# openxrlab/xrslam

Hardware: AMD Instinct MI355X
Metric: frames/sec, full per-frame hot path (KLT tracker + sliding-window VI-BA), one sequence per GPU (higher is better)
Workload: dtype u8/i16 images, f32 LK with exact i64 reductions, f64 BA

## Files before the change

xrslam_amd/csrc/ba_api.hip:

```cpp
#include "../../include/xrslam_hip.h"
#include "ba_kernels.hip.h"
#include "ba_chain.hip.h"
#include "ba_plan.hpp"
#include "ba_stage.hpp"
#include "marg_kernels.hip.h"
#include "cov_kernels.hip.h"
#include "host/covariance.hpp"
#include "common.hip.h"
#include "group.hip.h"

#include <cstdlib>
#include <chrono>
#include <algorithm>
#include <cmath>
#include <cstring>
#include <limits>
#include <vector>

using namespace xrhip;

namespace {

struct Grow {
    size_t headroom, floor;
// ... 81 lines not shown
        bool pending = false;
        int K = 0, victim = 0, R = 0;
        std::vector<double> lin;
        int *dst = nullptr;
        double *lam = nullptr;
    } marg;
    int preint_pending = 0;
    PreintScratch preint_o{};
    int preint_deferred = 0, preint_def_jac = 0, preint_def_cov = 0;
    bool profiling = false;
    struct Timed {
        hipEvent_t e0, e1;
        double flops_fixed, flops_per_trial;
        int iter_before;
    };
    std::vector<Timed> pending;
    struct TimedChain {
        hipEvent_t e0, e1;
        double bytes;
    };
    std::vector<TimedChain> pending_chain;
    std::vector<std::pair<hipEvent_t, hipEvent_t>> free_events;
    xrhip_ba_stats stats = {0, 0, 0.0, 0, 0.0, 0, 0, 0.0, 0.0, 0};
    DevBuf<> cov_dev;
    hipEvent_t cov_ev[5] = {nullptr, nullptr, nullptr, nullptr, nullptr};
    double cov_ms[4] = {0.0, 0.0, 0.0, 0.0};
    const TinyArgs *tiny_args = nullptr;
    hipStream_t stream2 = nullptr;
    hipEvent_t ev_mid = nullptr, ev_spec = nullptr;
    hipEvent_t ev_marg = nullptr;
    DevBuf<> work_spec;
    bool spec_outstanding = false;
    long spec_launched = 0, spec_taken = 0;
    const uint4 *stage_src = nullptr;
    uint4 *stage_dst = nullptr;
    size_t stage_n16 = 0;
    void (*overlap_fn)(void *) = nullptr;
    void *overlap_arg = nullptr;
    PinnedBuf<double> h_out;
    int lds_limit = 150 * 1024;
    int schur_mode = 0;
    SolvePlan plan;
};

static int ensure_arena(xrhip_ba *c, size_t in_bytes, size_t work_bytes, size_t out_doubles) {
    int rc = c->in.dev.reserve(in_bytes, GROW_DOUBLE_1M);
    if (!rc) rc = c->in.host.reserve(in_bytes, GROW_DOUBLE_1M);
    if (!rc) rc = c->work.reserve(work_bytes, GROW_DOUBLE_1M);
    if (!rc) rc = c->h_out.reserve(sizeof(double) * out_doubles, GROW_DOUBLE);
    return rc;
}

static int validate(const xrhip_ba_problem *P) {
    if (!P || P->n_frames <= 0 || !P->frame_state || !P->frame_fix) return xr_fail(XRHIP_EINVAL, "xrhip_ba_solve: frames missing");
    if (P->n_landmarks < 0 || P->n_obs < 0 || P->n_rot < 0 || P->n_imu < 0 || P->prior_n < 0)
        return xr_fail(XRHIP_EINVAL, "xrhip_ba_solve: negative count");
    for (int o = 0; o < P->n_obs; ++o)
        if (P->obs_tgt[o] < 0 || P->obs_tgt[o] >= P->n_frames || P->obs_ref[o] < 0 || P->obs_ref[o] >= P->n_frames ||
            P->obs_lm[o] < 0 || P->obs_lm[o] >= P->n_landmarks || P->obs_tgt[o] == P->obs_ref[o])
            return xr_fail(XRHIP_EINVAL, "xrhip_ba_solve: observation index out of range");
    for (int o = 0; o < P->n_rot; ++o)
        if (P->rot_tgt[o] < 0 || P->rot_tgt[o] >= P->n_frames || P->rot_ref[o] < 0 || P->rot_ref[o] >= P->n_frames)
            return xr_fail(XRHIP_EINVAL, "xrhip_ba_solve: rotation factor index out of range");
    for (int k = 0; k < P->n_imu; ++k)
        if (P->imu_i[k] < 0 || P->imu_i[k] >= P->n_frames || P->imu_j[k] < 0 || P->imu_j[k] >= P->n_frames ||
            P->imu_i[k] == P->imu_j[k])
// ... 195 lines not shown
    c->stage_n16 = (lay.in_bytes + 15) / 16;
    return defer_copy ? XRHIP_OK : launch_stage_copy(c, c->stream);
}

static int landmark_vision_blocks(const BaDims &d) { return d.lm_rows + d.F * d.F * VIS_CH; }
static int assemble_blocks(const BaDims &d) { return (d.n * d.n + 255) / 256; }
static size_t lin_all_lds(const BaDims &d) { return sizeof(double) * (size_t)std::max(d.np, 1); }
static int schur_aux_blocks(const BaDims &d) {
    const int tiles = d.PF / 16;
    const int nrest = sred_rest_blocks(d);
    return nrest + (d.nla ? tiles * tiles + aux_quad_blocks_n(d.n, d.L) + aux_wog_blocks(d.F) : aux_quad_blocks_n(d.n, d.L)) + 1;
}

static void launch_linearize(xrhip_ba *c, const Staged &st, bool for_solver) {
    hipStream_t s = c->stream;
    const BaDims &d = st.d;
    const BaPtrs &p = st.p;
    hipLaunchKernelGGL(kb_lin_all, dim3(lin_all_blocks(d.M, d.MR, d.NI, d.np)), dim3(256), lin_all_lds(d), s, d, p, st.cam, st.imu, st.sx, st.sy);
    hipLaunchKernelGGL(kb_landmark_vision, dim3(landmark_vision_blocks(d)), dim3(64), 0, s, d, p);
    if (for_solver && st.pl.route == ROUTE_SMALL_MID) return;
    hipLaunchKernelGGL(kb_assemble, dim3(assemble_blocks(d)), dim3(256), 0, s, d, p);
    if (for_solver) hipLaunchKernelGGL(kb_prepare, dim3(1), dim3(256), 0, s, d, p);
    else hipLaunchKernelGGL(kb_sum_cost, dim3(1), dim3(256), 0, s, d, p);
}

constexpr int LINEARIZE_LAUNCHES = 4;

static void launch_schur_aux(const Staged &st, hipStream_t s) {
    hipLaunchKernelGGL(kb_schur_aux, dim3(schur_aux_blocks(st.d)), dim3(256), 0, s, st.d, st.p);
}
static void launch_prior_lambda(const Staged &st, hipStream_t s) {
    hipLaunchKernelGGL(kb_prior_lambda, dim3(prior_lambda_blocks(st.d.np)), dim3(256), 0, s, st.d.np, st.p.pS, st.p.pLam, st.p.pinfo, st.p.pc0);
}
static void launch_trials_wide(const Staged &st, hipStream_t s, int seq, int first, int mode) {
    hipLaunchKernelGGL(kb_trials_wide, dim3(WIDE_G), dim3(256), st.pl.wide_lds, s, st.d, st.p, st.cam, st.imu, st.sx, st.sy, seq, first, mode);
}

static int take_event_pair(xrhip_ba *c, hipEvent_t *e0, hipEvent_t *e1) {
    if (!c->free_events.empty()) {
        *e0 = c->free_events.back().first;
        *e1 = c->free_events.back().second;
        c->free_events.pop_back();
    } else {
        XR_HIP(hipEventCreate(e0));
        XR_HIP(hipEventCreate(e1));
    }
    return XRHIP_OK;
}

static int launch_solve_try(xrhip_ba *c, const Staged &st, bool prepare, int mode, int seq, bool skip_front = false,
                            const BaPtrs *spec_set = nullptr) {
    const BaDims &d = st.d;
    const BaPtrs &p = st.p;
    const SolvePlan &pl = st.pl;
    const bool mark_mid = spec_set != nullptr;
    const int commit = (spec_set && skip_front) ? 1 : 0;
    double *state2 = spec_set ? static_cast<double *>(spec_set->state) : nullptr;
    double *depth2 = spec_set ? static_cast<double *>(spec_set->depth) : nullptr;
    BaCtl *ctl2 = spec_set ? static_cast<BaCtl *>(spec_set->ctl) : nullptr;
    hipStream_t s = c->stream;
    const bool mid = pl.route == ROUTE_SMALL_MID;
    if (!skip_front) {
        if (mid) hipLaunchKernelGGL(kb_small_mid, dim3(1), dim3(256), 0, s, d, p, prepare ? 0 : 1);
        if (!mid && prepare) hipLaunchKernelGGL(kb_prepare, dim3(1), dim3(256), 0, s, d, p);
        if (!mid) launch_schur_aux(st, s);
    }
    const size_t lds = pl.try_lds;
    const int use_lds = pl.use_lds, wide = pl.wide_trials ? 1 : 0;
// ... 8 lines not shown
    else if (pl.block == 256)
        hipLaunchKernelGGL((kb_solve_try<256, false>), dim3(1), dim3(256), lds, s, d, p, st.cam, st.imu, st.sx, st.sy, use_lds, mode, seq, wide,
                           (double *)nullptr, (double *)nullptr, (BaCtl *)nullptr, 0);
    else
        hipLaunchKernelGGL((kb_solve_try<512, false>), dim3(1), dim3(512), lds, s, d, p, st.cam, st.imu, st.sx, st.sy, use_lds, mode, seq, wide,
                           (double *)nullptr, (double *)nullptr, (BaCtl *)nullptr, 0);
    XR_HIP(hipGetLastError());
    if (c->profiling) XR_HIP(hipEventRecord(e1, s));
    if (pl.wide_first) {
        hipStream_t ts = s;
        if (mark_mid) {
            XR_HIP(hipEventRecord(c->ev_mid, s));
            XR_HIP(hipStreamWaitEvent(c->stream2, c->ev_mid, 0));
            ts = c->stream2;
        }
        launch_trials_wide(st, ts, seq, 1, mode);
        XR_HIP(hipGetLastError());
    }
    if (c->profiling) {
        const double na = d.na;
        c->pending.push_back({e0, e1, na * na * na / 3.0 + 2.0 * na * na,
                              pl.wide_first ? 0.0 : 450.0 * d.M + 3000.0 * d.NI + 2.0 * (double)d.np * d.np, -1});
    }
    c->stats.n_solve_try++;
    return XRHIP_OK;
}

static void run_overlap(xrhip_ba *c) {
    if (!c->overlap_fn) return;
    void (*fn)(void *) = c->overlap_fn;
    c->overlap_fn = nullptr;
    fn(c->overlap_arg);
}
static int wait_mailbox(xrhip_ba *c, int seq, hipStream_t publisher = nullptr, GroupRequest *rq = nullptr) {
    run_overlap(c);
    return wait_flag(c->h_seq, seq, publisher ? publisher : c->stream, rq, "xrhip_ba_solve");
}

static long long g_kprof[32];
static void kprof_accumulate(const BaCtl &ctl, int na) {
    static const int min_na = std::getenv("XRHIP_KPROF_MIN_NA") ? std::atoi(std::getenv("XRHIP_KPROF_MIN_NA")) : 0;
    static const int max_na = std::getenv("XRHIP_KPROF_MAX_NA") ? std::atoi(std::getenv("XRHIP_KPROF_MAX_NA")) : 1 << 30;
    if (na < min_na || na > max_na) return;
    for (int i = 0; i < 31; ++i) g_kprof[i] += ctl.prof[i];
    g_kprof[31] += 1;
}

extern "C" {

static void ba_resolve_pending(xrhip_ba *c) {
    for (auto &t : c->pending) {
        float ms = 0.f;
        if (hipEventSynchronize(t.e1) == hipSuccess && hipEventElapsedTime(&ms, t.e0, t.e1) == hipSuccess) {
            c->stats.ms_solve_try += ms;
            c->stats.n_timed += 1;
            c->stats.flops_solve_try += t.flops_fixed + t.flops_per_trial * std::max(t.iter_before, 0);
        }
        c->free_events.push_back({t.e0, t.e1});
    }
    c->pending.clear();
    for (auto &t : c->pending_chain) {
        float ms = 0.f;
        if (hipEventSynchronize(t.e1) == hipSuccess && hipEventElapsedTime(&ms, t.e0, t.e1) == hipSuccess) {
            c->stats.ms_chain += ms;
            c->stats.n_chain_timed += 1;
            c->stats.bytes_chain += t.bytes;
        }
        c->free_events.push_back({t.e0, t.e1});
    }
// ... 3 lines not shown
int xrhip_ba_set_profiling(xrhip_ba *c, int enable) {
    if (!c) return xr_fail(XRHIP_EINVAL, "xrhip_ba_set_profiling: null context");
    if (!enable) ba_resolve_pending(c);
    c->profiling = enable != 0;
    return XRHIP_OK;
}

int xrhip_ba_get_stats(xrhip_ba *c, xrhip_ba_stats *out, int reset) {
    if (!c || !out) return xr_fail(XRHIP_EINVAL, "xrhip_ba_get_stats: null argument");
    ba_resolve_pending(c);
    *out = c->stats;
    if (reset) c->stats = {0, 0, 0.0, 0, 0.0, 0, 0, 0.0, 0.0, 0};
    return XRHIP_OK;
}

void xrhip_debug_kprof(long long *out32, int reset) {
    for (int i = 0; i < 32; ++i) {
        if (out32) out32[i] = g_kprof[i];
        if (reset) g_kprof[i] = 0;
    }
}

int xrhip_ba_create(int max_frames, int max_landmarks, int max_obs, xrhip_ba **out) {
    if (!out || max_frames <= 0 || max_landmarks < 0 || max_obs < 0) return xr_fail(XRHIP_EINVAL, "xrhip_ba_create: bad arguments");
    int rc = xr_require_device();
    if (rc) return rc;
    xrhip_ba *c = new xrhip_ba();
    XR_HIP(hipGetDevice(&c->device));
    XR_HIP(hipStreamCreateWithFlags(&c->stream, hipStreamNonBlocking));
    XR_HIP(hipStreamCreateWithFlags(&c->stream2, hipStreamNonBlocking));
    XR_HIP(hipEventCreateWithFlags(&c->ev_mid, hipEventDisableTiming));
    XR_HIP(hipEventCreateWithFlags(&c->ev_spec, hipEventDisableTiming));
    XR_HIP(hipHostMalloc(&c->h_ctl, sizeof(BaCtl), hipHostMallocDefault));
    XR_HIP(hipHostMalloc(&c->h_seq, 64, hipHostMallocDefault));
    *c->h_seq = 0;
    XR_HIP(hipFuncSetAttribute((const void *)kb_solve_try<512, true>, hipFuncAttributeMaxDynamicSharedMemorySize, c->lds_limit));
    XR_HIP(hipFuncSetAttribute((const void *)kb_solve_try<512, false>, hipFuncAttributeMaxDynamicSharedMemorySize, c->lds_limit));
    XR_HIP(hipFuncSetAttribute((const void *)kb_solve_try<256, false>, hipFuncAttributeMaxDynamicSharedMemorySize, c->lds_limit));
    XR_HIP(hipFuncSetAttribute((const void *)kb_chain, hipFuncAttributeMaxDynamicSharedMemorySize, c->lds_limit));
    XR_HIP(hipFuncSetAttribute((const void *)kb_trials_wide, hipFuncAttributeMaxDynamicSharedMemorySize, c->lds_limit));
    XR_HIP(hipFuncSetAttribute((const void *)kw_solve_try, hipFuncAttributeMaxDynamicSharedMemorySize, c->lds_limit));
    XR_HIP(hipFuncSetAttribute((const void *)kw_trials_wide, hipFuncAttributeMaxDynamicSharedMemorySize, c->lds_limit));
    XR_HIP(hipFuncSetAttribute((const void *)km_chol, hipFuncAttributeMaxDynamicSharedMemorySize, c->lds_limit));
    XR_HIP(hipFuncSetAttribute((const void *)km_jacobi, hipFuncAttributeMaxDynamicSharedMemorySize, c->lds_limit));
    size_t in_guess = (size_t)max_obs * 96 + (size_t)max_frames * max_frames * 15 * 15 * 8 + (size_t)max_frames * 3000 + 65536;
    rc = ensure_arena(c, in_guess, in_guess * 4, (size_t)16 * max_frames + max_landmarks + 8);
    if (rc) return rc;
    *out = c;
    return XRHIP_OK;
}

int xrhip_ba_join_group(xrhip_ba *c, xrhip_group *g) {
    if (!c) return xr_fail(XRHIP_EINVAL, "xrhip_ba_join_group: null context");
    if (c->group == g) return XRHIP_OK;
    if (g && group_device(g) != c->device)
        return xr_fail(XRHIP_EINVAL, "xrhip_ba_join_group: the context and the group live on different devices");
    if (c->preint_pending) {
        if (c->preint_rq) {
            int rc = group_wait_launched(c->preint_rq);
            if (rc) return rc;
        }
        XR_HIP(hipStreamSynchronize(c->preint_stream ? c->preint_stream : c->stream));
        c->preint_rq = nullptr;
        c->preint_stream = c->stream;
    }
    XR_HIP(hipStreamSynchronize(c->stream));
    if (c->group) {
        int rc = group_drain(c->group, GQ_CHAIN, c);
        if (!rc) rc = group_drain(c->group, GQ_PREINT, c);
        if (!rc) rc = group_drain(c->group, GQ_WINDOW, c);
        if (rc) return rc;
        group_member_remove(c->group, false);
    }
    c->group = g;
    if (g) group_member_add(g, false);
    return XRHIP_OK;
}

void xrhip_ba_destroy(xrhip_ba *c) {
    if (!c) return;
    if (c->begun.active) xrhip_ba_solve_abort(c);
    if (c->group) {
        xrhip_ba_preintegrate_cancel(c);
        xrhip_ba_join_group(c, nullptr);
    }
    hipStreamSynchronize(c->stream);
    if (c->stream2) hipStreamSynchronize(c->stream2);
    if (std::getenv("XRHIP_HOSTPROF") && c->spec_launched)
        std::fprintf(stderr, "[hostprof] speculative linearisations: %ld launched, %ld taken\n", c->spec_launched, c->spec_taken);
    c->work_spec.release();
    c->cov_dev.release();
    for (hipEvent_t e : c->cov_ev)
        if (e) hipEventDestroy(e);
    if (c->ev_mid) hipEventDestroy(c->ev_mid);
    if (c->ev_marg) hipEventDestroy(c->ev_marg);
    if (c->ev_spec) hipEventDestroy(c->ev_spec);
    if (c->stream2) hipStreamDestroy(c->stream2);
    c->in.dev.release();
    c->in.host.release();
    c->work.release();
    c->work2.release();
    c->h_stage.release();
    hipHostFree(c->h_ctl);
    hipHostFree(c->h_seq);
    ba_resolve_pending(c);
    for (auto &e : c->free_events) {
        hipEventDestroy(e.first);
        hipEventDestroy(e.second);
    }
    c->h_out.release();
    hipStreamDestroy(c->stream);
    delete c;
}

static int preint_launch_deferred(xrhip_ba *c, const xrhip_ba_problem *P, const double *state_dev);
static int preint_fill_deferred(xrhip_ba *c, const xrhip_ba_problem *P, const double *state_dev, PreintArgs *out, bool *have);

static int ba_solve_impl(xrhip_ba *c, const xrhip_ba_problem *P, xrhip_ba_summary *summary);
int xrhip_ba_solve(xrhip_ba *c, const xrhip_ba_problem *P, xrhip_ba_summary *summary) {
    if (!c) return xr_fail(XRHIP_EINVAL, "xrhip_ba_solve: null context");
    if (c->begun.active) return xr_fail(XRHIP_ESTATE, "xrhip_ba_solve: a solve begun on this context has not been collected (xrhip_ba_solve_end)");
    const int rc = ba_solve_impl(c, P, summary);
// ... 211 lines not shown
    return XRHIP_OK;
}

int xrhip_ba_solve_chained(xrhip_ba *c1, const xrhip_ba_problem *P1, xrhip_ba_summary *s1, int link_first, xrhip_ba *c2,
                           const xrhip_ba_problem *P2, xrhip_ba_summary *s2, int link_second, void (*host_work)(void *), void *arg) {
    if (!c1 || !c2 || c1 == c2 || !P1 || !P2) return xr_fail(XRHIP_EINVAL, "xrhip_ba_solve_chained: two distinct contexts and two problems are needed");
    int rc = validate(P1);
    if (!rc) rc = validate(P2);
    if (rc) return rc;
    if (link_first < 0 || link_first >= P1->n_frames || link_second < 0 || link_second >= P2->n_frames)
        return xr_fail(XRHIP_EINVAL, "xrhip_ba_solve_chained: linked frame is not a frame of its problem");
    const int begun = xrhip_ba_solve_begin(c1, P1);
    if (begun < 0) return begun;
    if (begun == 0) {
        rc = xrhip_ba_solve_overlapped(c1, P1, s1, host_work, arg);
        if (rc) return rc;
        std::memcpy(P2->frame_state + 16 * (size_t)link_second, P1->frame_state + 16 * (size_t)link_first, sizeof(double) * 16);
        return xrhip_ba_solve(c2, P2, s2);
    }
    rc = xrhip_ba_solve_linked(c2, P2, s2, link_second, c1, link_first, host_work, arg);
    const int rc1 = xrhip_ba_solve_end(c1, s1);
    return rc ? rc : rc1;
}

struct RoundIssuer {
    enum Form { OWN, SPEC, GROUP };
    xrhip_ba *c;
    Staged &st;
    Form form;
    hipStream_t wstream;
    Staged st2{};
    bool spec_ready = false;
    bool first = true, relin = true;

    int begin_spec() {
        const int rc = c->work_spec.reserve(c->work.cap + spec_extra_bytes(st.d), GROW_EXACT);
        if (rc) return rc;
        st2 = st;
        st2.p = spec_set(st.p, st.d, c->work.p, c->work_spec.p, c->work.cap);
        return XRHIP_OK;
    }
    int request(int kind, int seq, int mode) {
        int r = group_wait_launched(&c->rq_window);
        if (r) return r;
        const BaDims &d = st.d;
        WindowPayload &wp = c->a_window;
        wp.e = WinEntry{c->tiny_args, lin_all_blocks(d.M, d.MR, d.NI, d.np), landmark_vision_blocks(d), assemble_blocks(d), schur_aux_blocks(d),
                        st.pl.use_lds, mode, seq, 1};
        wp.relin = relin;
        wp.with_stage = first;
        wp.stage = StageArgs{c->stage_src, c->stage_dst, c->stage_n16};
        wp.np = d.np;
        wp.pS = st.p.pS;
        wp.pLam = st.p.pLam;
        wp.pinfo = st.p.pinfo;
        wp.pc0 = st.p.pc0;
        wp.lds_lin = lin_all_lds(d);
        wp.lds_solve = st.pl.try_lds;
        wp.lds_wide = st.pl.wide_lds;
        c->rq_window.kind = kind;
        c->rq_window.owner = c;
        c->rq_window.payload = &wp;
        first = false;
        return group_submit(c->group, GQ_WINDOW, &c->rq_window);
    }
    int round(bool relinearise, int mode, int seq) {
        relin = relinearise;
        if (form == GROUP) return request(GK_WROUND, seq, mode);
        int rc;
        if (spec_ready) {
            rc = launch_solve_try(c, st, false, mode, seq, true, &st2.p);
        } else {
            if (relinearise) launch_linearize(c, st, true);
            rc = launch_solve_try(c, st, !relinearise, mode, seq, false, form == SPEC ? &st2.p : nullptr);
        }
        if (rc) return rc;
        spec_ready = false;
        if (form == SPEC) {
            launch_linearize(c, st2, true);
            launch_schur_aux(st2, c->stream);
            XR_HIP(hipGetLastError());
            c->spec_launched++;
        }
        return XRHIP_OK;
    }
    int trials(int seq) {
        if (form == GROUP) return request(GK_WTRIALS, seq, 0);
        launch_trials_wide(st, form == SPEC ? c->stream2 : c->stream, seq, 0, 0);
        XR_HIP(hipGetLastError());
        return XRHIP_OK;
    }
    int wait(int seq) {
        if (form == GROUP) return wait_mailbox(c, seq, wstream, &c->rq_window);
        return wait_mailbox(c, seq, form == SPEC ? c->stream2 : nullptr);
    }
    void costed(int n_trials) {
        if (c->profiling && form != GROUP && !c->pending.empty()) c->pending.back().iter_before = n_trials;
    }
    void take_speculation() {
        if (form != SPEC) return;
        swap_lin_sets(st.p, st2.p);
        spec_ready = true;
        c->spec_taken++;
    }
};

static int ba_solve_impl(xrhip_ba *c, const xrhip_ba_problem *P, xrhip_ba_summary *summary) {
    int rc = validate(P);
    if (rc) return rc;
    rc = preint_deferred_check(c, P);
    if (rc) return rc;
    c->plan = SolvePlan{};
    c->plan.F = P->n_frames;
    bool any_free = any_free_block(P);
    if (!any_free) {
        std::vector<char> used(std::max(P->n_landmarks, 1), 0);
        for (int o = 0; o < P->n_obs; ++o) used[P->obs_lm[o]] = 1;
        for (int l = 0; l < P->n_landmarks; ++l)
            if (used[l] && !(P->landmark_fix && P->landmark_fix[l])) any_free = true;
    }
    if (!any_free) {
        if (summary) {
            std::memset(summary, 0, sizeof(*summary));
            summary->termination = XRHIP_BA_CONVERGENCE;
            summary->usable = 1;
        }
        return preint_launch_deferred(c, P, nullptr);
// ... 27 lines not shown
    const BaSwitches &sw = ba_switches();
    const bool wbatch = c->group && !sw.group_no_window_batch && pl.wide_first && d.nla > 0 && !sw.group_spec;
    const bool spec = !sw.no_spec && pl.wide_first && !(c->group && !sw.group_spec);
    if (!wbatch) {
        rc = launch_stage_copy(c, c->stream);
        if (rc) return rc;
    }
    if (!d.nla) st.d.lm_rows = 0;
    if (d.np && !wbatch) launch_prior_lambda(st, c->stream);
    RoundIssuer rounds{c, st, wbatch ? RoundIssuer::GROUP : spec ? RoundIssuer::SPEC : RoundIssuer::OWN,
                       wbatch ? group_stream(c->group, GQ_WINDOW) : nullptr};
    bool done = false;
    struct BusyElsewhere {
        xrhip_group *g;
        explicit BusyElsewhere(xrhip_group *gg) : g(gg) { group_busy_elsewhere(g, 1); }
        ~BusyElsewhere() { group_busy_elsewhere(g, -1); }
    } busy_elsewhere(c->group);
    if (pl.route == ROUTE_TINY) {
        const int seq = ++c->seq;
        hipLaunchKernelGGL(kb_tiny, dim3(1), dim3(256), pl.try_lds, c->stream, c->tiny_args, pl.use_lds, seq, 4 * (P->max_iterations + 8));
        XR_HIP(hipGetLastError());
        rc = wait_mailbox(c, seq);
        if (rc) return rc;
        if (c->h_ctl->status != ST_DONE) return xr_fail(XRHIP_ESTATE, "xrhip_ba_solve: trust-region loop did not terminate");
        c->stats.n_tiny++;
        done = true;
    }
    if (rounds.form == RoundIssuer::SPEC) {
        rc = rounds.begin_spec();
        if (rc) return rc;
    }
    bool relinearise = true;
    int mode = 1, iter_seen = 0;
    auto trials_since = [&]() {
        const int it_now = c->h_ctl->iteration, trials = std::max(0, it_now - iter_seen);
        iter_seen = it_now;
        c->stats.n_trials += trials;
        return trials;
    };
    for (int guard = 0; guard < 4 * (P->max_iterations + 8) && !done; ++guard) {
        const int seq = ++c->seq;
        rc = rounds.round(relinearise, mode, seq);
        if (!rc) rc = rounds.wait(seq);
        if (rc) return rc;
        const bool first_batch_accept = c->h_ctl->status == ST_ACCEPTED && c->h_ctl->accepted_slot == 0;
        rounds.costed(trials_since());
        int status = c->h_ctl->status;
        for (int wguard = 0; status == ST_NEED_TRIALS && wguard < 64; ++wguard) {
            const int wseq = ++c->seq;
            rc = rounds.trials(wseq);
            if (!rc) rc = rounds.wait(wseq);
            if (rc) return rc;
            trials_since();
            status = c->h_ctl->status;
        }
        if (status == ST_DONE) {
            done = true;
        } else if (status == ST_ACCEPTED) {
            relinearise = true;
            mode = 1;
            if (first_batch_accept) rounds.take_speculation();
        } else if (status == ST_RESOLVE || status == ST_RESOLVE_INNER) {
            relinearise = false;
            mode = (status == ST_RESOLVE) ? 2 : 3;
        } else {
            return xr_fail(XRHIP_ESTATE, "xrhip_ba_solve: unexpected device status");
        }
    }
    if (!done) return xr_fail(XRHIP_ESTATE, "xrhip_ba_solve: trust-region loop did not terminate");
    std::memcpy(P->frame_state, c->h_out.p, sizeof(double) * 16 * d.F);
    if (d.L && d.nla) std::memcpy(P->inv_depth, c->h_out.p + 16 * d.F, sizeof(double) * d.L);
    rc = preint_launch_deferred(c, P, nullptr);
    if (rc) return rc;
    kprof_accumulate(*c->h_ctl, d.na);
    fill_summary(*c->h_ctl, ms_since(t_begin), summary);
    return XRHIP_OK;
}

int xrhip_ba_debug_marg_guard(xrhip_ba *c, double *lambda_bound, int *status8) {
    if (!c || !lambda_bound || !status8) return xr_fail(XRHIP_EINVAL, "xrhip_ba_debug_marg_guard: null argument");
    if (c->marg.pending || !c->marg.lam) return xr_fail(XRHIP_ESTATE, "xrhip_ba_debug_marg_guard: no collected marginalisation on this context");
    XR_HIP(hipStreamSynchronize(c->stream));
    XR_HIP(hipMemcpy(lambda_bound, c->marg.lam, sizeof(double), hipMemcpyDeviceToHost));
    XR_HIP(hipMemcpy(status8, c->marg.dst, sizeof(int) * 8, hipMemcpyDeviceToHost));
    return XRHIP_OK;
}

int xrhip_ba_debug_set_schur_precision(xrhip_ba *c, int mode) {
    if (!c || mode < 0 || mode > 2) return xr_fail(XRHIP_EINVAL, "xrhip_ba_debug_set_schur_precision: bad arguments");
    c->schur_mode = mode;
    return XRHIP_OK;
}

int xrhip_ba_debug_last_route(xrhip_ba *c, int *out8) {
    if (!c || !out8) return xr_fail(XRHIP_EINVAL, "xrhip_ba_debug_last_route: null argument");
    const SolvePlan &pl = c->plan;
    const int route[8] = {pl.route, pl.use_lds, pl.sred_tiled, pl.block, pl.wide_trials ? 1 : 0, pl.wide_first ? 1 : 0, pl.na, pl.F};
    std::memcpy(out8, route, sizeof(route));
    return XRHIP_OK;
}

int xrhip_ba_debug_linearize(xrhip_ba *c, const xrhip_ba_problem *P, double *H, double *g, double *hll, double *gl,
// ... 503 lines not shown
```

xrslam_amd/csrc/ba_kernels.hip.h:

```cpp
#pragma once
#include <hip/hip_runtime.h>
#include <stdint.h>

#include "ba_math.hip.h"
#include "batch.hip.h"
#include "dense_lds.hip.h"

namespace xrhip {

constexpr int OREC = 28;
constexpr int RREC = 8;
constexpr int TRY_B = 4;
constexpr int WIDE_B = 8;
constexpr int WIDE_G = 64;
constexpr int QF_ROWS = 8;

struct BaCtl {
    double radius, mu;
    double x_cost, cand_cost, minimum_cost;
    double x_norm, gmax, alpha, step_norm;
    double model_cost_change, initial_cost;
    double q_gg, q_gn, q_nn;
    double gnorm, gn_norm, gd;
    int iteration, successful_steps, invalid_steps;
    int reuse;
    int status;
    int termination;
    int linear_ok;
    int first;
    int max_iterations;
    unsigned wide_ticket;
    int accepted_slot;
    long long prof[32];
};
#ifdef XRHIP_KPROF
#define KPROF_BEGIN() long long kp_t = wall_clock64()
#define KPROF(slot)                                                   \
    do {                                                              \
        __syncthreads();                                              \
        if (threadIdx.x == 0) {                                       \
            const long long kp_n = wall_clock64();                    \
            p.ctl->prof[slot] += kp_n - kp_t;                         \
            kp_t = kp_n;                                              \
        }                                                             \
    } while (0)
#else
#define KPROF_BEGIN() \
    do {              \
    } while (0)
#define KPROF(slot) \
    do {            \
    } while (0)
#endif
enum { ST_RUNNING = 0, ST_ACCEPTED = 1, ST_RESOLVE = 2, ST_DONE = 3, ST_NEED_TRIALS = 4, ST_RESOLVE_INNER = 102 };

struct BaDims {
    int F, n, PF;
    int L, Lp;
    int M, MR, NI;
    int NP, np;
    int NV;
    int robust;
    int na;
    int nla;
    int lm_rows;
    int nfree;
    int nffp;
    int schur_mode;
    int sred_tiled;
};

template <class T> struct gptr {
    __attribute__((address_space(1))) T *raw;
    __host__ __device__ __forceinline__ operator T *() const { return (T *)raw; }
    __host__ __device__ __forceinline__ T *operator->() const { return (T *)raw; }
    __host__ __device__ __forceinline__ gptr &operator=(T *p) {
        raw = (__attribute__((address_space(1))) T *)p;
        return *this;
    }
};

struct BaPtrs {
    gptr<double> state, cand;
    gptr<const uint8_t> fix;
    gptr<double> depth, depth_cand;
    gptr<const uint8_t> lact;
    gptr<const int> obs_tgt, obs_ref, obs_lm;
// ... 1368 lines not shown
            t.status = ST_RESOLVE;
        }
        return false;
    }
    if (w.dn <= TR_PARAMETER_TOLERANCE * (t.x_norm + TR_PARAMETER_TOLERANCE) ||
        fabs(t.x_cost - w.cost) <= TR_FUNCTION_TOLERANCE * t.x_cost) {
        t.termination = XRHIP_BA_CONVERGENCE;
        t.status = ST_DONE;
        return false;
    }
    if (w.relative_decrease > TR_MIN_RELATIVE_DECREASE) {
        t.invalid_steps = 0;
        t.successful_steps += 1;
        if (w.relative_decrease < 0.25) t.radius *= 0.5;
        if (w.relative_decrease > 0.75) t.radius = fmax(t.radius, 3.0 * step_norm);
        t.radius = fmin(t.radius, TR_MAX_RADIUS);
        t.mu = fmax(1e-8, 2.0 * t.mu / 10.0);
        t.reuse = 0;
        t.cand_cost = w.cost;
        t.last_step_norm = step_norm;
        t.status = ST_ACCEPTED;
        return true;
    }
    t.invalid_steps = 0;
    t.radius *= 0.5;
    t.reuse = 1;
    return false;
}
__device__ __forceinline__ bool trial_decide(TrialScalars &t, int k, double model_cost_change, double cost, double dn2,
                                             double step_norm) {
    return trial_decide(t, k, model_cost_change, trial_terms(t, model_cost_change, cost, dn2), step_norm);
}

__device__ __forceinline__ void publish_block(const BaDims &d, const BaPtrs &p, int status, int seq, bool always) {
    const int tid = threadIdx.x, nt = blockDim.x;
    if (status == ST_DONE) {
        for (int e = tid; e < 16 * d.F; e += nt) p.host_out[e] = p.state[e];
        for (int l = tid; l < d.L; l += nt) p.host_out[16 * d.F + l] = p.depth[l];
        __threadfence_system();
    }
    if (tid == 0) p.ctl->status = status;
    __syncthreads();
    if (always || status == ST_DONE) {
        constexpr unsigned ctl_words = sizeof(BaCtl) / sizeof(long long);
        long long *src = reinterpret_cast<long long *>(static_cast<BaCtl *>(p.ctl));
        long long *dst = reinterpret_cast<long long *>(static_cast<BaCtl *>(p.host_ctl));
        for (unsigned i = tid; i < ctl_words; i += nt) dst[i] = __hip_atomic_load(src + i, __ATOMIC_RELAXED, __HIP_MEMORY_SCOPE_AGENT);
        __threadfence_system();
        __syncthreads();
        if (tid == 0) *reinterpret_cast<volatile int *>(static_cast<int *>(p.host_seq)) = seq;
    }
    __syncthreads();
}

__device__ __forceinline__ int try_block(const BaDims &d, const BaPtrs &p, const Ext &cam, const Ext &imu, double sx,
                                         double sy, int after_linearisation, int seq, bool wide_after_first, double *sh,
                                         bool prep_only = false, bool publish_always = true) {
    __shared__ double scratch[2 * TRY_B * 8];
    BaCtl *c = p.ctl;
    const int tid = threadIdx.x, nt = blockDim.x;

    const int mode = after_linearisation;
    KPROF_BEGIN();
    if (mode == 1) {
        for (int k = tid; k < d.NI; k += nt) {
            const double *st = p.state + 16 * p.imu_i[k];
            for (int i = 0; i < 6; ++i) p.bias_ref[6 * k + i] = st[10 + i];
        }
        const double xn2 = ambient_norm2(d, p, p.state, p.depth, scratch);
        if (tid == 0) {
            c->x_norm = sqrt(xn2);
            c->first = 0;
        }
        __syncthreads();
    }
    KPROF(10);
// ... 179 lines not shown
#pragma unroll
            for (int q = 0; q < TRY_B; ++q)
                if (q == k) red[2 * q + 1] += df * df;
        }
        if (B == 1) {
            double r1[2] = {red[0], red[1]};
            block_sum_n<2>(r1, scratch);
            red[0] = r1[0];
            red[1] = r1[1];
        } else {
            block_sum_n<2 * TRY_B>(red, scratch);
        }
        KPROF(18);
        int accepted = -1;
#pragma unroll
        for (int k = 0; k < TRY_B; ++k) {
            if (k >= B || t.status != ST_RUNNING) continue;
#ifdef XRHIP_KPROF
            if (tid == 0) p.ctl->prof[19] += 1;
#endif
            if (trial_decide(t, k, model_cost_change[k], red[2 * k], red[2 * k + 1], step_norm[k])) accepted = k;
        }
        if (accepted >= 0) {
            const double *cs = p.cand + (size_t)accepted * 16 * d.F, *cd = p.depth_cand + (size_t)accepted * d.L;
            for (int e = tid; e < 16 * d.F; e += nt) p.state[e] = cs[e];
            for (int l = tid; l < d.L; l += nt) p.depth[l] = cd[l];
        }
        __syncthreads();
        if (t.status == ST_RUNNING && wide_after_first) t.status = ST_NEED_TRIALS;
        B = TRY_B;
    }
    if (tid == 0) trial_store(c, t);
    __syncthreads();
    publish_block(d, p, t.status, seq, publish_always);
    return t.status;
}


__device__ __forceinline__ void d_lin_all(const BaDims &d, const BaPtrs &p, const Ext &cam, const Ext &imu, double sx, double sy, int bx) {
    extern __shared__ double sh[];
    __shared__ double scr[IMU_SCR + IMU_XCH];
    __shared__ double scratch[8];
    const int nbo = (d.M + 255) / 256, nbr = (d.MR + 255) / 256, nbi = d.NI;
    int blk = bx;
    if (blk < nbo) {
        const int o = blk * 256 + threadIdx.x;
        if (o < d.M) lin_obs_item(d, p, cam, sx, sy, o);
        return;
    }
    blk -= nbo;
    if (blk < nbr) {
        const int o = blk * 256 + threadIdx.x;
        if (o < d.MR) lin_rot_item(d, p, cam, sx, sy, o);
        return;
    }
    blk -= nbr;
    if (blk < nbi) {
        lin_imu_block(d, p, imu, blk, scr);
        return;
    }
    blk -= nbi;
    if (d.NP == 0) {
        if (threadIdx.x == 0) p.pcost[0] = 0.0;
        return;
    }
    lin_prior_rows_block(d, p, blk, sh, scratch);
}
// ... 48 lines not shown
}
template <int NT, bool PREP>
__device__ __forceinline__ void d_solve_try(const BaDims &d, const BaPtrs &p, const Ext &cam, const Ext &imu, double sx, double sy, int use_lds,
                                            int after_linearisation, int seq, int wide_trials, double *state2, double *depth2,
                                            BaCtl *ctl2, int commit) {
    extern __shared__ double lds[];
    if (PREP && commit) {
        if (threadIdx.x == 0) {
            p.ctl->x_cost = ctl2->x_cost;
            p.ctl->gmax = ctl2->gmax;
        }
        __syncthreads();
    }
    solve_block(d, p, use_lds, lds);
    __syncthreads();
    if (PREP) {
        try_block(d, p, cam, imu, sx, sy, after_linearisation, seq, true, lds, true);
        if (state2) {
            __syncthreads();
            spec_state_block(d, p, state2, depth2, ctl2, after_linearisation);
        }
    } else {
        try_block(d, p, cam, imu, sx, sy, after_linearisation, seq, wide_trials != 0, lds, false);
    }
}
template <int NT, bool PREP>
__global__ __launch_bounds__(NT) void kb_solve_try(BaDims d, BaPtrs p, Ext cam, Ext imu, double sx, double sy, int use_lds,
                                                   int after_linearisation, int seq, int wide_trials, double *state2, double *depth2,
                                                   BaCtl *ctl2, int commit) {
    d_solve_try<NT, PREP>(d, p, cam, imu, sx, sy, use_lds, after_linearisation, seq, wide_trials, state2, depth2, ctl2, commit);
}

__device__ __forceinline__ void d_trials_wide(const BaDims &d, const BaPtrs &p, const Ext &cam, const Ext &imu, double sx, double sy, int seq,
                                              int first, int mode, int bx, int gx) {
    extern __shared__ double wl[];
    __shared__ double scratch[4 * WIDE_B * 4];
    __shared__ int s_last;
    const int tid = threadIdx.x, nt = blockDim.x, lane = tid & 63, wave = tid >> 6, nw = nt >> 6;
    const int blk = bx, G = gx;
    const int n = d.n;
#ifdef XRHIP_KPROF_PRINT
    long long tw[16];
    int twn = 0;
#define WT() (tw[twn++] = wall_clock64())
#else
#define WT() ((void)0)
#endif
    WT();
    double *cand = wl;
    double *pd = wl + (size_t)WIDE_B * 16 * d.F;
    BaCtl *c = p.ctl;
    TrialScalars t;
    trial_load(c, t);
    if (first) {
        trial_begin(t, mode == 3, mode == 1);
        if (t.status != ST_RUNNING) {
            if (blk == 0) {
                if (tid == 0) trial_store(c, t);
                __syncthreads();
                publish_block(d, p, t.status, seq, true);
            }
            return;
        }
    }
    int dup = 0;
    {
        double rk = t.radius;
        while (dup < 60 && t.gn_norm <= rk) {
            ++dup;
            rk *= 0.5;
        }
        if (dup < 1) dup = 1;
    }
    double ca[WIDE_B], cb[WIDE_B], step_norm[WIDE_B];
#pragma unroll
    for (int k = 0; k < WIDE_B; ++k) {
        const int j = k == 0 ? 0 : dup + k - 1;
        dogleg_point(t, scalbn(t.radius, -j), ca[k], cb[k], step_norm[k]);
    }
    WT();
    for (int e = tid; e < WIDE_B * d.F; e += nt) {
        const int k = e / d.F, f = e - k * d.F;
        double dl[15];
#pragma unroll
        for (int q = 0; q < 15; ++q) {
            const int a = 15 * f + q;
            double cak = 0, cbk = 0;
#pragma unroll
            for (int kk = 0; kk < WIDE_B; ++kk)
                if (kk == k) {
                    cak = ca[kk];
                    cbk = cb[kk];
                }
// ... 181 lines not shown
#pragma unroll
    for (int k = 1; k < WIDE_B; ++k) {
        if (t.status != ST_RUNNING) continue;
        const int jj = dup + k - 1;
        if (trial_decide(t, first ? jj : jj + 1, mcc[k], terms[k], step_norm[k])) accepted = k;
#ifdef XRHIP_KPROF
        ++decisions;
#endif
    }
#ifdef XRHIP_KPROF
    if (tid == 0) p.ctl->prof[19] += decisions;
#endif
    WT();
    if (accepted >= 0) {
        for (int e = tid; e < 16 * d.F; e += nt) p.state[e] = cand[(size_t)accepted * 16 * d.F + e];
        double cak = 0, cbk = 0;
#pragma unroll
        for (int kk = 0; kk < WIDE_B; ++kk)
            if (kk == accepted) {
                cak = ca[kk];
                cbk = cb[kk];
            }
        for (int l = tid; l < d.L; l += nt)
            if (p.lact[l]) p.depth[l] = p.depth[l] + ((cak * p.grad[n + l] + cbk * p.gn[n + l]) / p.diagD[n + l]) * p.sl[l];
    }
    if (t.status == ST_RUNNING) t.status = ST_NEED_TRIALS;
    if (tid == 0) {
        trial_store(c, t);
        c->wide_ticket = 0;
        c->accepted_slot = accepted;
    }
    __syncthreads();
    WT();
    publish_block(d, p, t.status, seq, true);
#ifdef XRHIP_KPROF_PRINT
    if (tid == 0 && d.M > 1500)
        printf("kb_trials_wide LAST block %d: load+dogleg %lld cand %lld prior_delta %lld nv %lld obs+rot %lld imu %lld prior %lld reduce %lld ticket %lld fence+sum %lld decide %lld apply %lld publish %lld (x10ns)\n", blk,
               tw[1] - tw[0], tw[2] - tw[1], tw[3] - tw[2], tw[4] - tw[3], tw[5] - tw[4], tw[6] - tw[5], tw[7] - tw[6], tw[8] - tw[7], tw[9] - tw[8],
               tw[10] - tw[9], tw[11] - tw[10], tw[12] - tw[11], wall_clock64() - tw[12]);
#endif
#undef WT
}
__global__ __launch_bounds__(256) void kb_trials_wide(BaDims d, BaPtrs p, Ext cam, Ext imu, double sx, double sy, int seq,
                                                      int first, int mode) {
    d_trials_wide(d, p, cam, imu, sx, sy, seq, first, mode, blockIdx.x, gridDim.x);
}

__device__ __forceinline__ void small_mid_block(const BaDims &d, const BaPtrs &p, int relinearised, double *scratch) {
    const int tid = threadIdx.x, nt = blockDim.x, lane = tid & 63, wave = tid >> 6, nw = nt >> 6;
    const int n = d.n, na = d.na;
    if (relinearised) {
        const bool col0_active = dof_active(p.fix, 0);
        for (int e = tid; e < na * (na + 1); e += nt) {
            const int i = e / (na + 1), j = e - i * (na + 1);
            if (j == na && col0_active) continue;
            assemble_item(d, p, p.act_idx[i] * n + (j < na ? p.act_idx[j] : 0));
        }
        for (int a = tid; a < n; a += nt)
            if (!dof_active(p.fix, a)) {
                p.Hpp[(size_t)a * n + a] = 0.0;
                p.gp[a] = 0.0;
            }
        __syncthreads();
        sum_cost_block(d, p, scratch);
        __syncthreads();
        gradmax_block(d, p, scratch);
    }
    prepare_block(d, p);
    __syncthreads();
    for (int blk = 0; blk < sred_rest_blocks(d); ++blk) reduced_rest_block(d, p, blk);
    double acc = 0;
    for (int i = wave; i < na; i += nw) {
        const int a = p.act_idx[i];
        const double Da = p.diagD[a], ga = p.sp[a] * (p.gs[a] / (Da * Da));
        double t = 0;
        for (int j = lane; j < na; j += 64) {
            const int b = p.act_idx[j];
            const double Db = p.diagD[b];
// ... 195 lines not shown
```

xrslam_amd/csrc/ba_plan.hpp:

```cpp
#pragma once
#include "../../include/xrslam_hip.h"
#include "ba_kernels.hip.h"
#include "ba_chain.hip.h"

#include <algorithm>
#include <cstdlib>

namespace xrhip {

struct BaSwitches {
    bool no_tiny = false;
    bool no_chain = false;
    bool no_obs_cache = false;
    bool no_tiled = false;
    bool no_spec = false;
    bool group_spec = false;
    bool group_no_window_batch = false;
    bool no_chained_solves = false;
    bool group_chained_solves = false;
};
inline const BaSwitches &ba_switches() {
    auto set = [](const char *name) { return std::getenv(name) != nullptr; };
    static const BaSwitches s = {set("XRHIP_NO_TINY"),   set("XRHIP_NO_CHAIN"),   set("XRHIP_NO_OBS_CACHE"),
                                 set("XRHIP_NO_TILED"),  set("XRHIP_NO_SPEC"),    set("XRHIP_GROUP_SPEC"),
                                 set("XRHIP_GROUP_NO_WINDOW_BATCH"), set("XRHIP_NO_CHAINED_SOLVES"), set("XRHIP_GROUP_CHAINED_SOLVES")};
    return s;
}

enum BaRoute { ROUTE_NONE = 0, ROUTE_TINY = 1, ROUTE_CHAIN = 2, ROUTE_SMALL_MID = 3, ROUTE_MULTI = 4 };

struct SolvePlan {
    int route = ROUTE_NONE;
    int na = 0, F = 0;
    size_t chain_lds = 0;
    int chain_opts = 0;
    int use_lds = -1;
    int sred_tiled = 0;
    size_t try_lds = 0;
    int block = 0;
    bool wide_trials = false;
    bool wide_first = false;
    size_t wide_lds = 0;
};

inline SolvePlan plan_solve(const BaDims &d, size_t lds_limit, const BaSwitches &sw) {
    SolvePlan pl;
    pl.na = d.na;
    pl.F = d.F;
    const size_t tri = (size_t)(d.na + 1) * (d.na + 2) / 2;
    const size_t tiled = (size_t)tl_doubles(d.na + 1) + 16 * (size_t)tl_tile_rows(d.na + 1);
    const size_t aux = (size_t)d.PF;
    size_t lds = sizeof(double) * std::max(tiled, aux);
    int use_lds = 2;
    if (sw.no_tiled || lds > lds_limit) {
        lds = sizeof(double) * std::max(tri, aux);
        use_lds = 1;
    }
    if (lds > lds_limit) {
        use_lds = 0;
// ... 40 lines not shown
```

xrslam_amd/csrc/group.hip.h:

```cpp
#pragma once
#include <hip/hip_runtime.h>

#include <atomic>
#include <functional>

#include "../../include/xrslam_hip.h"

namespace xrhip {

enum GroupQueue { GQ_KLT = 0, GQ_CHAIN, GQ_PREINT, GQ_WINDOW, GQ_COUNT };
enum GroupKind { GK_CALL = 0, GK_UPLOAD, GK_PREPROCESS, GK_TRACK, GK_DETECT, GK_CHAIN, GK_PREINT, GK_WROUND, GK_WTRIALS, GK_COUNT };
constexpr int GK_GATE_SLOT = 11;

struct GroupRequest {
    int kind = GK_CALL;
    void *owner = nullptr;
    void *payload = nullptr;
    std::function<int(hipStream_t)> call;
    std::atomic<int> state{0};
    int rc = 0;
    char err[256] = {0};
};

typedef int (*GroupLaunchFn)(GroupRequest **reqs, int n, hipStream_t s, hipStream_t side);
void group_register(int kind, GroupLaunchFn fn);

int group_submit(xrhip_group *g, int queue, GroupRequest *r);
int group_wait_launched(GroupRequest *r);
int group_call(xrhip_group *g, int queue, void *owner, std::function<int(hipStream_t)> fn);
int group_drain(xrhip_group *g, int queue, void *owner);
hipStream_t group_stream(xrhip_group *g, int queue);
int group_device(xrhip_group *g);
hipStream_t group_side_stream(xrhip_group *g, int queue);
void group_member_add(xrhip_group *g, bool front_end);
void group_member_remove(xrhip_group *g, bool front_end);
void group_busy_elsewhere(xrhip_group *g, int delta);

void group_gate_register(xrhip_group *g, void *owner);
void group_gate_unregister(xrhip_group *g, void *owner);
void group_gate_busy(xrhip_group *g, void *owner, bool busy);
void group_gate_arrive(xrhip_group *g, void *owner);

int wait_flag(volatile int *flag, int seq, hipStream_t s, GroupRequest *req, const char *what, hipStream_t s2 = nullptr);

}
```

xrslam_amd/csrc/group_api.hip:

```cpp
#include "group.hip.h"

#include "common.hip.h"

#include <cstdio>
#include <chrono>
#include <condition_variable>
#include <deque>
#include <mutex>
#include <thread>
#include <vector>
#if defined(__x86_64__)
#include <immintrin.h>
#endif

using namespace xrhip;

namespace {

GroupLaunchFn g_launch[GK_COUNT] = {nullptr};

inline void relax() {
#if defined(__x86_64__)
    _mm_pause();
#else
// ... 340 lines not shown
        g->gate_used.store(true, std::memory_order_relaxed);
        me->absent = false;
        my_gen = g->gate_gen.load(std::memory_order_relaxed);
        me->arrived_gen = my_gen;
        if (g->gate_ready_locked()) {
            g->gate_full++;
            g->gate_timeouts_in_a_row = 0;
            g->gate_open_locked();
            return;
        }
        g->gate_recount_locked();
    }
    const auto t0 = std::chrono::steady_clock::now();
    for (unsigned spin = 1;; ++spin) {
        if (g->gate_gen.load(std::memory_order_acquire) != my_gen) return;
        relax();
        if ((spin & 63) != 0) continue;
        if (std::chrono::steady_clock::now() - t0 < std::chrono::microseconds(g->gate_timeout_us)) continue;
        std::lock_guard<std::mutex> lk(g->gate_m);
        if (g->gate_gen.load(std::memory_order_relaxed) != my_gen) return;
        for (xrhip_group::GateMember &m : g->gate_members)
            if (!m.busy && !m.absent && m.arrived_gen != my_gen) m.absent = true;
        g->gate_timeouts++;
        if (++g->gate_timeouts_in_a_row >= 16) {
            g->gate_on.store(false);
            g->gate_used.store(false, std::memory_order_relaxed);
            g->linger_us.store(0, std::memory_order_relaxed);
        }
        g->gate_open_locked();
        return;
    }
}

int wait_flag(volatile int *flag, int seq, hipStream_t s, GroupRequest *req, const char *what, hipStream_t s2) {
    if (req) {
        const int rc = group_wait_launched(req);
        if (rc) return rc;
    }
    for (unsigned long spin = 1;; ++spin) {
        if (*flag == seq) return XRHIP_OK;
        if ((spin & 0x3FFF) == 0) {
            hipError_t q = hipStreamQuery(s);
            if (q == hipSuccess && s2) q = hipStreamQuery(s2);
            if (q == hipSuccess) {
                if (*flag == seq) return XRHIP_OK;
                std::snprintf(xr_err_buf(), 512, "%s: kernel retired without publishing its result", what);
                return XRHIP_ESTATE;
            }
            if (q != hipErrorNotReady) {
                (void)hipGetLastError();
                std::snprintf(xr_err_buf(), 512, "%s: stream error while waiting for the kernel", what);
                return XRHIP_EHIP;
            }
        }
    }
}

}

extern "C" {

int xrhip_group_create(xrhip_group **out) {
    if (!out) return xr_fail(XRHIP_EINVAL, "xrhip_group_create: null argument");
    int rc = xr_require_device();
    if (rc) return rc;
    xrhip_group *g = new xrhip_group();
    std::memset(&g->stats, 0, sizeof(g->stats));
    hipGetDevice(&g->device);
    if (const char *e = std::getenv("XRHIP_GROUP_GATE")) g->gate_on.store(std::atoi(e) != 0);
    if (const char *e = std::getenv("XRHIP_GROUP_GATE_TIMEOUT_US")) g->gate_timeout_us = std::max(1, std::atoi(e));
    g->linger_us.store(g->gate_on.load() ? 40 : 0);
    if (const char *e = std::getenv("XRHIP_GROUP_LINGER_US")) g->linger_us.store(std::max(0, std::atoi(e)));
    if (const char *e = std::getenv("XRHIP_GROUP_LINGER_QUEUES")) g->linger_queues = std::atoi(e);
    if (const char *e = std::getenv("XRHIP_GROUP_PER_KIND")) g->per_kind = std::atoi(e) != 0;
    int prio_low = 0, prio_high = 0;
    const char *qe = std::getenv("GPU_MAX_HW_QUEUES"), *pe = std::getenv("XRHIP_GROUP_PRIORITY");
    const bool want_prio = pe ? std::atoi(pe) != 0 : (qe && std::atoi(qe) > 0 && std::atoi(qe) <= 2);
    const bool use_prio = want_prio && hipDeviceGetStreamPriorityRange(&prio_low, &prio_high) == hipSuccess && prio_high != prio_low;
// ... 99 lines not shown
```

Measured before the change: 1629.

## Queue next trial batch speculatively before host reads the trust-region decision

Each round now launches the next kb_trials_wide batch immediately, guarded on the device by an expected decided_seq and ST_NEED_TRIALS status, so the GPU need not wait for a host round trip between trial batches. Kernels publish a per-sequence decision record into a double-buffered mailbox, and the host reads the decision from that record instead of the shared ctl block. This hides launch latency in the trial loop. In exchange, a batch is wasted whenever the solve does not need more trials, and failure paths must drain both streams.

```diff
diff --git a/xrslam_amd/csrc/ba_api.hip b/xrslam_amd/csrc/ba_api.hip
--- a/xrslam_amd/csrc/ba_api.hip
+++ b/xrslam_amd/csrc/ba_api.hip
@@ -137,6 +137,7 @@
     DevBuf<> work_spec;
     bool spec_outstanding = false;
     long spec_launched = 0, spec_taken = 0;
+    long ahead_issued = 0, ahead_skipped = 0;
     const uint4 *stage_src = nullptr;
     uint4 *stage_dst = nullptr;
     size_t stage_n16 = 0;
@@ -398,8 +399,9 @@
 static void launch_prior_lambda(const Staged &st, hipStream_t s) {
     hipLaunchKernelGGL(kb_prior_lambda, dim3(prior_lambda_blocks(st.d.np)), dim3(256), 0, s, st.d.np, st.p.pS, st.p.pLam, st.p.pinfo, st.p.pc0);
 }
-static void launch_trials_wide(const Staged &st, hipStream_t s, int seq, int first, int mode) {
-    hipLaunchKernelGGL(kb_trials_wide, dim3(WIDE_G), dim3(256), st.pl.wide_lds, s, st.d, st.p, st.cam, st.imu, st.sx, st.sy, seq, first, mode);
+static void launch_trials_wide(const Staged &st, hipStream_t s, int seq, int first, int mode, int expect_seq = 0) {
+    hipLaunchKernelGGL(kb_trials_wide, dim3(WIDE_G), dim3(256), st.pl.wide_lds, s, st.d, st.p, st.cam, st.imu, st.sx, st.sy, seq, first, mode,
+                       expect_seq);
 }
 
 static int take_event_pair(xrhip_ba *c, hipEvent_t *e0, hipEvent_t *e1) {
@@ -474,9 +476,9 @@
     c->overlap_fn = nullptr;
     fn(c->overlap_arg);
 }
-static int wait_mailbox(xrhip_ba *c, int seq, hipStream_t publisher = nullptr, GroupRequest *rq = nullptr) {
+static int wait_mailbox(xrhip_ba *c, int seq, hipStream_t publisher = nullptr, GroupRequest *rq = nullptr, bool or_later = false) {
     run_overlap(c);
-    return wait_flag(c->h_seq, seq, publisher ? publisher : c->stream, rq, "xrhip_ba_solve");
+    return wait_flag(c->h_seq, seq, publisher ? publisher : c->stream, rq, "xrhip_ba_solve", nullptr, or_later);
 }
 
 static long long g_kprof[32];
@@ -546,8 +548,8 @@
     XR_HIP(hipEventCreateWithFlags(&c->ev_mid, hipEventDisableTiming));
     XR_HIP(hipEventCreateWithFlags(&c->ev_spec, hipEventDisableTiming));
     XR_HIP(hipHostMalloc(&c->h_ctl, sizeof(BaCtl), hipHostMallocDefault));
-    XR_HIP(hipHostMalloc(&c->h_seq, 64, hipHostMallocDefault));
-    *c->h_seq = 0;
+    XR_HIP(hipHostMalloc(&c->h_seq, sizeof(int) * MB_INTS, hipHostMallocDefault));
+    std::memset(c->h_seq, 0, sizeof(int) * MB_INTS);
     XR_HIP(hipFuncSetAttribute((const void *)kb_solve_try<512, true>, hipFuncAttributeMaxDynamicSharedMemorySize, c->lds_limit));
     XR_HIP(hipFuncSetAttribute((const void *)kb_solve_try<512, false>, hipFuncAttributeMaxDynamicSharedMemorySize, c->lds_limit));
     XR_HIP(hipFuncSetAttribute((const void *)kb_solve_try<256, false>, hipFuncAttributeMaxDynamicSharedMemorySize, c->lds_limit));
@@ -602,6 +604,9 @@
     if (c->stream2) hipStreamSynchronize(c->stream2);
     if (std::getenv("XRHIP_HOSTPROF") && c->spec_launched)
         std::fprintf(stderr, "[hostprof] speculative linearisations: %ld launched, %ld taken\n", c->spec_launched, c->spec_taken);
+    if (std::getenv("XRHIP_HOSTPROF") && c->ahead_issued)
+        std::fprintf(stderr, "[hostprof] trial batches queued ahead of the decision: %ld launched, %ld ran, %ld skipped (not trials, not timed)\n",
+                     c->ahead_issued, c->ahead_issued - c->ahead_skipped, c->ahead_skipped);
     c->work_spec.release();
     c->cov_dev.release();
     for (hipEvent_t e : c->cov_ev)
@@ -879,6 +884,41 @@
     Staged st2{};
     bool spec_ready = false;
     bool first = true, relin = true;
+    bool ahead = false;
+    int ahead_seq = 0;
+    struct Decision {
+        int status, slot, iteration;
+    };
+
+    hipStream_t trial_stream() const { return form == SPEC ? c->stream2 : c->stream; }
+    void queue_ahead(int behind_seq) {
+        ahead_seq = ++c->seq;
+        launch_trials_wide(st, trial_stream(), ahead_seq, 0, 0, behind_seq);
+        c->ahead_issued++;
+    }
+    int decision(int seq, Decision &out) const {
+        if (!ahead) {
+            out = Decision{c->h_ctl->status, c->h_ctl->accepted_slot, c->h_ctl->iteration};
+            return XRHIP_OK;
+        }
+        const volatile int *rec = c->h_seq + MB_REC0 + MB_REC_INTS * (seq & 1);
+        if (rec[0] != seq) return xr_fail(XRHIP_ESTATE, "xrhip_ba_solve: the mailbox holds no decision record of the awaited launch");
+        out = Decision{rec[1], rec[2], rec[3]};
+        return XRHIP_OK;
+    }
+    void settle() {
+        if (ahead_seq) c->ahead_skipped++;
+        ahead_seq = 0;
+    }
+    int fail(int rc) {
+        if (ahead) {
+            (void)hipStreamSynchronize(c->stream);
+            (void)hipStreamSynchronize(trial_stream());
+            (void)hipGetLastError();
+            ahead_seq = 0;
+        }
+        return rc;
+    }
 
     int begin_spec() {
         const int rc = c->work_spec.reserve(c->work.cap + spec_extra_bytes(st.d), GROW_EXACT);
@@ -929,17 +969,28 @@
             XR_HIP(hipGetLastError());
             c->spec_launched++;
         }
+        if (ahead) {
+            queue_ahead(seq);
+            XR_HIP(hipGetLastError());
+        }
         return XRHIP_OK;
     }
-    int trials(int seq) {
+    int trials(int &seq) {
+        if (ahead) {
+            seq = ahead_seq;
+            queue_ahead(seq);
+            XR_HIP(hipGetLastError());
+            return XRHIP_OK;
+        }
+        seq = ++c->seq;
         if (form == GROUP) return request(GK_WTRIALS, seq, 0);
-        launch_trials_wide(st, form == SPEC ? c->stream2 : c->stream, seq, 0, 0);
+        launch_trials_wide(st, trial_stream(), seq, 0, 0);
         XR_HIP(hipGetLastError());
         return XRHIP_OK;
     }
     int wait(int seq) {
         if (form == GROUP) return wait_mailbox(c, seq, wstream, &c->rq_window);
-        return wait_mailbox(c, seq, form == SPEC ? c->stream2 : nullptr);
+        return wait_mailbox(c, seq, form == SPEC ? c->stream2 : nullptr, nullptr, ahead);
     }
     void costed(int n_trials) {
         if (c->profiling && form != GROUP && !c->pending.empty()) c->pending.back().iter_before = n_trials;
@@ -1033,28 +1084,33 @@
     }
     bool relinearise = true;
     int mode = 1, iter_seen = 0;
-    auto trials_since = [&]() {
-        const int it_now = c->h_ctl->iteration, trials = std::max(0, it_now - iter_seen);
+    auto trials_since = [&](int it_now) {
+        const int trials = std::max(0, it_now - iter_seen);
         iter_seen = it_now;
         c->stats.n_trials += trials;
         return trials;
     };
+    rounds.ahead = !done && rounds.form != RoundIssuer::GROUP && pl.wide_trials && !ba_host_driven();
+    RoundIssuer::Decision dec{};
     for (int guard = 0; guard < 4 * (P->max_iterations + 8) && !done; ++guard) {
         const int seq = ++c->seq;
         rc = rounds.round(relinearise, mode, seq);
         if (!rc) rc = rounds.wait(seq);
-        if (rc) return rc;
-        const bool first_batch_accept = c->h_ctl->status == ST_ACCEPTED && c->h_ctl->accepted_slot == 0;
-        rounds.costed(trials_since());
-        int status = c->h_ctl->status;
+        if (!rc) rc = rounds.decision(seq, dec);
+        if (rc) return rounds.fail(rc);
+        const bool first_batch_accept = dec.status == ST_ACCEPTED && dec.slot == 0;
+        rounds.costed(trials_since(dec.iteration));
+        int status = dec.status;
         for (int wguard = 0; status == ST_NEED_TRIALS && wguard < 64; ++wguard) {
-            const int wseq = ++c->seq;
+            int wseq = 0;
             rc = rounds.trials(wseq);
             if (!rc) rc = rounds.wait(wseq);
-            if (rc) return rc;
-            trials_since();
-            status = c->h_ctl->status;
-        }
+            if (!rc) rc = rounds.decision(wseq, dec);
+            if (rc) return rounds.fail(rc);
+            trials_since(dec.iteration);
+            status = dec.status;
+        }
+        if (status != ST_NEED_TRIALS) rounds.settle();
         if (status == ST_DONE) {
             done = true;
         } else if (status == ST_ACCEPTED) {
@@ -1065,10 +1121,10 @@
             relinearise = false;
             mode = (status == ST_RESOLVE) ? 2 : 3;
         } else {
-            return xr_fail(XRHIP_ESTATE, "xrhip_ba_solve: unexpected device status");
-        }
-    }
-    if (!done) return xr_fail(XRHIP_ESTATE, "xrhip_ba_solve: trust-region loop did not terminate");
+            return rounds.fail(xr_fail(XRHIP_ESTATE, "xrhip_ba_solve: unexpected device status"));
+        }
+    }
+    if (!done) return rounds.fail(xr_fail(XRHIP_ESTATE, "xrhip_ba_solve: trust-region loop did not terminate"));
     std::memcpy(P->frame_state, c->h_out.p, sizeof(double) * 16 * d.F);
     if (d.L && d.nla) std::memcpy(P->inv_depth, c->h_out.p + 16 * d.F, sizeof(double) * d.L);
     rc = preint_launch_deferred(c, P, nullptr);
diff --git a/xrslam_amd/csrc/ba_kernels.hip.h b/xrslam_amd/csrc/ba_kernels.hip.h
--- a/xrslam_amd/csrc/ba_kernels.hip.h
+++ b/xrslam_amd/csrc/ba_kernels.hip.h
@@ -31,6 +31,7 @@
     int max_iterations;
     unsigned wide_ticket;
     int accepted_slot;
+    int decided_seq;
     long long prof[32];
 };
 #ifdef XRHIP_KPROF
@@ -53,6 +54,7 @@
     } while (0)
 #endif
 enum { ST_RUNNING = 0, ST_ACCEPTED = 1, ST_RESOLVE = 2, ST_DONE = 3, ST_NEED_TRIALS = 4, ST_RESOLVE_INNER = 102 };
+constexpr int MB_REC0 = 4, MB_REC_INTS = 4, MB_INTS = 16;
 
 struct BaDims {
     int F, n, PF;
@@ -1487,16 +1489,26 @@
     return trial_decide(t, k, model_cost_change, trial_terms(t, model_cost_change, cost, dn2), step_norm);
 }
 
-__device__ __forceinline__ void publish_block(const BaDims &d, const BaPtrs &p, int status, int seq, bool always) {
+__device__ __forceinline__ void publish_block(const BaDims &d, const BaPtrs &p, int status, int seq, bool always, int iteration, int slot) {
     const int tid = threadIdx.x, nt = blockDim.x;
     if (status == ST_DONE) {
         for (int e = tid; e < 16 * d.F; e += nt) p.host_out[e] = p.state[e];
         for (int l = tid; l < d.L; l += nt) p.host_out[16 * d.F + l] = p.depth[l];
         __threadfence_system();
     }
-    if (tid == 0) p.ctl->status = status;
+    if (tid == 0) {
+        p.ctl->status = status;
+        p.ctl->decided_seq = seq;
+    }
     __syncthreads();
     if (always || status == ST_DONE) {
+        if (tid == nt - 1) {
+            volatile int *rec = static_cast<int *>(p.host_seq) + MB_REC0 + MB_REC_INTS * (seq & 1);
+            rec[0] = seq;
+            rec[1] = status;
+            rec[2] = slot;
+            rec[3] = iteration;
+        }
         constexpr unsigned ctl_words = sizeof(BaCtl) / sizeof(long long);
         long long *src = reinterpret_cast<long long *>(static_cast<BaCtl *>(p.ctl));
         long long *dst = reinterpret_cast<long long *>(static_cast<BaCtl *>(p.host_ctl));
@@ -1742,7 +1754,7 @@
     }
     if (tid == 0) trial_store(c, t);
     __syncthreads();
-    publish_block(d, p, t.status, seq, publish_always);
+    publish_block(d, p, t.status, seq, publish_always, t.iteration, -1);
     return t.status;
 }
 
@@ -1857,7 +1869,12 @@
 }
 
 __device__ __forceinline__ void d_trials_wide(const BaDims &d, const BaPtrs &p, const Ext &cam, const Ext &imu, double sx, double sy, int seq,
-                                              int first, int mode, int bx, int gx) {
+                                              int first, int mode, int bx, int gx, int expect_seq = 0) {
+    if (expect_seq) {
+        const int status = __hip_atomic_load(&p.ctl->status, __ATOMIC_RELAXED, __HIP_MEMORY_SCOPE_AGENT);
+        const int decided = __hip_atomic_load(&p.ctl->decided_seq, __ATOMIC_RELAXED, __HIP_MEMORY_SCOPE_AGENT);
+        if (status != ST_NEED_TRIALS || decided != expect_seq) return;
+    }
     extern __shared__ double wl[];
     __shared__ double scratch[4 * WIDE_B * 4];
     __shared__ int s_last;
@@ -1883,7 +1900,7 @@
             if (blk == 0) {
                 if (tid == 0) trial_store(c, t);
                 __syncthreads();
-                publish_block(d, p, t.status, seq, true);
+                publish_block(d, p, t.status, seq, true, t.iteration, -1);
             }
             return;
         }
@@ -2131,7 +2148,7 @@
     }
     __syncthreads();
     WT();
-    publish_block(d, p, t.status, seq, true);
+    publish_block(d, p, t.status, seq, true, t.iteration, accepted);
 #ifdef XRHIP_KPROF_PRINT
     if (tid == 0 && d.M > 1500)
         printf("kb_trials_wide LAST block %d: load+dogleg %lld cand %lld prior_delta %lld nv %lld obs+rot %lld imu %lld prior %lld reduce %lld ticket %lld fence+sum %lld decide %lld apply %lld publish %lld (x10ns)\n", blk,
@@ -2141,8 +2158,8 @@
 #undef WT
 }
 __global__ __launch_bounds__(256) void kb_trials_wide(BaDims d, BaPtrs p, Ext cam, Ext imu, double sx, double sy, int seq,
-                                                      int first, int mode) {
-    d_trials_wide(d, p, cam, imu, sx, sy, seq, first, mode, blockIdx.x, gridDim.x);
+                                                      int first, int mode, int expect_seq) {
+    d_trials_wide(d, p, cam, imu, sx, sy, seq, first, mode, blockIdx.x, gridDim.x, expect_seq);
 }
 
 __device__ __forceinline__ void small_mid_block(const BaDims &d, const BaPtrs &p, int relinearised, double *scratch) {
diff --git a/xrslam_amd/csrc/ba_plan.hpp b/xrslam_amd/csrc/ba_plan.hpp
--- a/xrslam_amd/csrc/ba_plan.hpp
+++ b/xrslam_amd/csrc/ba_plan.hpp
@@ -25,6 +25,10 @@
                                  set("XRHIP_NO_TILED"),  set("XRHIP_NO_SPEC"),    set("XRHIP_GROUP_SPEC"),
                                  set("XRHIP_GROUP_NO_WINDOW_BATCH"), set("XRHIP_NO_CHAINED_SOLVES"), set("XRHIP_GROUP_CHAINED_SOLVES")};
     return s;
+}
+inline bool ba_host_driven() {
+    const char *e = std::getenv("XRHIP_HOST_DRIVEN");
+    return e && e[0] && !(e[0] == '0' && !e[1]);
 }
 
 enum BaRoute { ROUTE_NONE = 0, ROUTE_TINY = 1, ROUTE_CHAIN = 2, ROUTE_SMALL_MID = 3, ROUTE_MULTI = 4 };
diff --git a/xrslam_amd/csrc/group.hip.h b/xrslam_amd/csrc/group.hip.h
--- a/xrslam_amd/csrc/group.hip.h
+++ b/xrslam_amd/csrc/group.hip.h
@@ -41,6 +41,6 @@
 void group_gate_busy(xrhip_group *g, void *owner, bool busy);
 void group_gate_arrive(xrhip_group *g, void *owner);
 
-int wait_flag(volatile int *flag, int seq, hipStream_t s, GroupRequest *req, const char *what, hipStream_t s2 = nullptr);
+int wait_flag(volatile int *flag, int seq, hipStream_t s, GroupRequest *req, const char *what, hipStream_t s2 = nullptr, bool or_later = false);
 
 }
diff --git a/xrslam_amd/csrc/group_api.hip b/xrslam_amd/csrc/group_api.hip
--- a/xrslam_amd/csrc/group_api.hip
+++ b/xrslam_amd/csrc/group_api.hip
@@ -396,18 +396,22 @@
     }
 }
 
-int wait_flag(volatile int *flag, int seq, hipStream_t s, GroupRequest *req, const char *what, hipStream_t s2) {
+int wait_flag(volatile int *flag, int seq, hipStream_t s, GroupRequest *req, const char *what, hipStream_t s2, bool or_later) {
     if (req) {
         const int rc = group_wait_launched(req);
         if (rc) return rc;
     }
+    auto reached = [&]() {
+        const int f = *flag;
+        return f == seq || (or_later && f - seq > 0);
+    };
     for (unsigned long spin = 1;; ++spin) {
-        if (*flag == seq) return XRHIP_OK;
+        if (reached()) return XRHIP_OK;
         if ((spin & 0x3FFF) == 0) {
             hipError_t q = hipStreamQuery(s);
             if (q == hipSuccess && s2) q = hipStreamQuery(s2);
             if (q == hipSuccess) {
-                if (*flag == seq) return XRHIP_OK;
+                if (reached()) return XRHIP_OK;
                 std::snprintf(xr_err_buf(), 512, "%s: kernel retired without publishing its result", what);
                 return XRHIP_ESTATE;
             }
```

Result: slower. 1599 (-1.8%).
